# stardist/stardist

Hardware: AMD Instinct MI355X
Metric: predict_instances() Mpix/s (2D) + Mvox/s (3D) end-to-end at 1/2/4/8 GPU (higher is better)
Workload: dtype f32

## Files before the change

stardist_amd/csrc/clip_beam.h:

```cpp
#pragma once
#include "clip_sweep.h"
#include <limits.h>

#if defined(BEAM_COUNT) && !defined(__HIP_DEVICE_COMPILE__)
struct BeamCounters { long beams, topx, isect_pt, isect_edges, outpt, update, maxima, lm, horz, ael_sum, il_beams, es_loads; };
inline BeamCounters& beam_counters() { static BeamCounters c = {}; return c; }
#define BEAM_CNT(f, v) (beam_counters().f += (v))
#else
#define BEAM_CNT(f, v) ((void)0)
#endif
#ifndef BEAM_PH
#define BEAM_PH(i) ((void)0)
#endif
enum { BEAM_PH_PREP = 0, BEAM_PH_SETUP, BEAM_PH_LM, BEAM_PH_POP, BEAM_PH_HORZ, BEAM_PH_ILIST, BEAM_PH_ISECT, BEAM_PH_TOP_EDGES, BEAM_PH_TOP_HORZ,
       BEAM_PH_TOP_UPDATE, BEAM_PH_END, BEAM_PH_COUNT };

namespace sdclip {

typedef unsigned long long u64;

enum {
  ST_OVERFLOW_AEL = 32,
  ST_OVERFLOW_LM = 64,
  ST_OVERFLOW_GJ = 128
};
enum { BEAM_MAXLM = 8 };

struct PrepPt { int x, y; };
template <bool WIDE> struct PrepIdx { typedef unsigned char type; enum { NONE = 255 }; };
template <> struct PrepIdx<true> { typedef unsigned short type; enum { NONE = 65535 }; };
template <int MAXV>
struct PolyPrep {
  typedef typename PrepIdx<(MAXV > 128)>::type pidx;
  enum { NONE = PrepIdx<(MAXV > 128)>::NONE };
  int n;
  int n_lm;
  int status;
  int pad;
  PrepPt v[MAXV + 1];
  unsigned char ecode[MAXV];
  pidx mpair[MAXV];
  pidx hlast[MAXV];
  pidx lm_left[BEAM_MAXLM], lm_right[BEAM_MAXLM];
};

#ifndef BEAM_PREP_IDX
#define BEAM_PREP_IDX short
#endif
template <class P, int MAXV>
struct PrepWork {
  typedef BEAM_PREP_IDX ridx;
  static constexpr unsigned RI = P::template region<int, MAXV>(), RS = P::template region<ridx, MAXV>(),
                            RB = P::template region<unsigned char, MAXV>();
  static constexpr unsigned O_CX = 0, O_CY = O_CX + RI, O_NXT = O_CY + RI, O_PRV = O_NXT + RS, O_CODE = O_PRV + RS,
                            O_N = O_CODE + RB, O_LMY = O_N + P::template region<int, 1>(), O_LML = O_LMY + P::template region<int, BEAM_MAXLM>(),
                            O_LMR = O_LML + P::template region<short, BEAM_MAXLM>(), O_END = O_LMR + P::template region<short, BEAM_MAXLM>();
  static constexpr unsigned lds_bytes() { return O_END; }
  typename P::template Arr<int, MAXV, O_CX> cx; typename P::template Arr<int, MAXV, O_CY> cy;
  typename P::template Arr<ridx, MAXV, O_NXT> nxt; typename P::template Arr<ridx, MAXV, O_PRV> prv;
  typename P::template Arr<unsigned char, MAXV, O_CODE> code;
  typename P::template Scalar<int, O_N> n;
  typename P::template Arr<int, BEAM_MAXLM, O_LMY> lmy;
  typename P::template Arr<short, BEAM_MAXLM, O_LML> lml_; typename P::template Arr<short, BEAM_MAXLM, O_LMR> lmr_;

  SD_HD int nx(int e) const { return e + 1 == n ? 0 : e + 1; }
  SD_HD int pv(int e) const { return e == 0 ? n - 1 : e - 1; }
  SD_HD bool sw(int e) const { return (code[e] & 4) != 0; }
  SD_HD int botx(int e) const { return sw(e) ? cx[nx(e)] : cx[e]; }
  SD_HD int boty(int e) const { return sw(e) ? cy[nx(e)] : cy[e]; }
  SD_HD int topx(int e) const { return sw(e) ? cx[e] : cx[nx(e)]; }
  SD_HD int topy(int e) const { return sw(e) ? cy[e] : cy[nx(e)]; }
  SD_HD bool is_horz(int e) const { return cy[e] == cy[nx(e)]; }
  SD_HD double dx(int e) const {
    const i64 dy = (i64)topy(e) - boty(e);
    if (dy == 0) return SD_HORIZONTAL;
    return (double)((i64)topx(e) - botx(e)) / (double)dy;
// ... 136 lines not shown
      if (n_lm < BEAM_MAXLM) {
        int k = n_lm;
        while (k > 0 && lmy[k - 1] < y) { lmy[k] = lmy[k - 1]; lml_[k] = lml_[k - 1]; lmr_[k] = lmr_[k - 1]; --k; }
        lmy[k] = y; lml_[k] = (short)left; lmr_[k] = (short)right;
        ++n_lm;
      } else st |= ST_OVERFLOW_LM;
      if (!leftFwd) E = E2;
    }
    for (int i = 0; i < m; ++i) { out->v[i].x = cx[i]; out->v[i].y = cy[i]; }
    out->v[m].x = cx[0]; out->v[m].y = cy[0];
    for (int i = 0; i < m; ++i) {
      const int c = code[i] & 3;
      const int nl = (c == 1) ? nx(i) : (c == 2 ? pv(i) : -1);
      int cc = code[i] & 7;
      if (nl >= 0 && is_horz(nl)) cc |= 8;
      out->ecode[i] = (unsigned char)cc;
      const int a = nx(i), b = pv(i);
      int mp = PolyPrep<MAXV>::NONE;
      if (topx(a) == topx(i) && topy(a) == topy(i) && (code[a] & 3) == 0) mp = a;
      else if (topx(b) == topx(i) && topy(b) == topy(i) && (code[b] & 3) == 0) mp = b;
      out->mpair[i] = (typename PolyPrep<MAXV>::pidx)mp;
      int last = i, g2 = 0;
      if (is_horz(i)) {
        for (;;) {
          const int c2 = code[last] & 3;
          const int n2 = (c2 == 1) ? nx(last) : (c2 == 2 ? pv(last) : -1);
          if (n2 < 0 || !is_horz(n2)) break;
          last = n2;
          if (++g2 > MAXV) { st |= ST_ITER; break; }
        }
      }
      out->hlast[i] = (typename PolyPrep<MAXV>::pidx)last;
    }
    for (int i = 0; i < n_lm; ++i) { out->lm_left[i] = (typename PolyPrep<MAXV>::pidx)lml_[i]; out->lm_right[i] = (typename PolyPrep<MAXV>::pidx)lmr_[i]; }
    out->n = m; out->n_lm = n_lm; out->status = st;
  }
};

template <class D, class P, int MAXV, int K, int MAXIL, bool FULLGJ = false>
struct BeamCore {
  typedef PolyPrep<MAXV> Prep;
  template <bool W, int = 0> struct OrdT { typedef unsigned int type; };
  template <int D0> struct OrdT<true, D0> { typedef u64 type; };
  typedef typename OrdT<(K > 8)>::type ord_t;
  enum { ORD_BITS = (K > 8) ? 64 : 32 };
  enum { GJ = (K <= 8 ? 3 : 4), NX = (K <= 8 ? 2 : 4), EID_POLY = 4096 };
  SD_HD D& self() { return *static_cast<D*>(this); }
  static constexpr unsigned RI = P::template coord_region<K>(), RD = P::template slope_region<K>(),
                            RS = P::template region<short, K>(), RB = P::template region<signed char, K>(),
                            RIL = P::template coord_region<MAXIL>(), RILB = P::template region<signed char, MAXIL>(),
                            RG = P::template coord_region<GJ>(), RGF = P::template region<int, (FULLGJ ? GJ : 1)>(), R1 = P::template region<int, 1>(), R8 = P::template region<u64, 1>(), RO = P::template region<ord_t, 1>();
  static constexpr unsigned O_BOTX = 0, O_BOTY = O_BOTX + RI, O_TOPX = O_BOTY + RI, O_TOPY = O_TOPX + RI, O_CURX = O_TOPY + RI,
                            O_DX = O_CURX + RI, O_EID = O_DX + RD, O_WCNT = O_EID + RS, O_WCNT2 = O_WCNT + RB,
                            O_OUTIDX = O_WCNT2 + RB, O_LMLC = O_OUTIDX + RB, O_WDELTA = O_LMLC + RB, O_PTYP = O_WDELTA + RB,
                            O_SIDE = O_PTYP + RB, O_ILX = O_SIDE + RB, O_ILY = O_ILX + RIL, O_ILE1 = O_ILY + RIL, O_ILE2 = O_ILE1 + RILB,
                            O_GJOP = O_ILE2 + RILB, O_GJX1 = O_GJOP + RGF, O_GJX2 = O_GJX1 + RG, O_GJY2 = O_GJX2 + RG,
                            O_XTRA = O_GJY2 + RGF, O_MLM = O_XTRA + P::template region<int, NX>(),
                            O_PA = O_MLM + P::template region<unsigned char, 16>(),
                            O_ORD = O_PA + 2 * R8, O_HSEL = O_ORD + RO, O_AFTER_ORD = O_HSEL + RO, O_PB = O_PA + R8, O_NAEL = O_AFTER_ORD, O_FREE = O_NAEL + R1, O_NLM = O_FREE + R1,
                            O_CURLM = O_NLM + R1, O_NIL = O_CURLM + R1, O_STATUS = O_NIL + R1, O_NJOINS = O_STATUS + R1,
                            O_NGJ = O_NJOINS + R1, O_NXTRA = O_NGJ + R1, O_LMY = O_NXTRA + R1, O_ORGX = O_LMY + R1, O_ORGY = O_ORGX + R1, O_SCANY = O_ORGY + R1, O_RINGN = O_SCANY + R1,
                            O_CORE_END = O_RINGN + P::template region<int, 2>();
  typename P::template CoordArr<K, O_BOTX, O_ORGX, O_STATUS> botx; typename P::template CoordArr<K, O_BOTY, O_ORGY, O_STATUS> boty;
  typename P::template CoordArr<K, O_TOPX, O_ORGX, O_STATUS> topx; typename P::template CoordArr<K, O_TOPY, O_ORGY, O_STATUS> topy;
  typename P::template CoordArr<K, O_CURX, O_ORGX, O_STATUS> curx;
  typename P::template SlopeArr<K, O_DX, O_BOTX, O_BOTY, O_TOPX, O_TOPY> dx;
  typename P::template Arr<short, K, O_EID> eid;
  typename P::template Arr<signed char, K, O_WCNT> wcnt; typename P::template Arr<signed char, K, O_WCNT2> wcnt2;
  typename P::template Arr<signed char, K, O_OUTIDX> outidx;
  typename P::template Arr<signed char, K, O_LMLC> lmlc;
  typename P::template Arr<signed char, K, O_WDELTA> wdelta; typename P::template Arr<signed char, K, O_PTYP> ptyp;
  typename P::template Arr<signed char, K, O_SIDE> side;
  typename P::template CoordArr<MAXIL, O_ILX, O_ORGX, O_STATUS> ilx; typename P::template CoordArr<MAXIL, O_ILY, O_ORGY, O_STATUS> ily;
  typename P::template Arr<signed char, MAXIL, O_ILE1> ile1; typename P::template Arr<signed char, MAXIL, O_ILE2> ile2;
  typename P::template Arr<int, (FULLGJ ? GJ : 1), O_GJOP> gjop; typename P::template CoordArr<GJ, O_GJX1, O_ORGX, O_STATUS> gjx1;
  typename P::template CoordArr<GJ, O_GJX2, O_ORGX, O_STATUS> gjx2; typename P::template Arr<int, (FULLGJ ? GJ : 1), O_GJY2> gjy2;
  typename P::template Arr<int, NX, O_XTRA> xtra;
  typename P::template Arr<unsigned char, 16, O_MLM> mlm;
  typename P::template Scalar<ord_t, O_ORD> ord;
  typename P::template Scalar<ord_t, O_HSEL> hsel;
  typename P::template Scalar<const Prep*, O_PA> prepA; typename P::template Scalar<const Prep*, O_PB> prepB;
  typename P::template Scalar<int, O_NAEL> n_ael; typename P::template Scalar<int, O_FREE> freemask;
  typename P::template Scalar<int, O_NLM> n_lm; typename P::template Scalar<int, O_CURLM> cur_lm;
  typename P::template Scalar<int, O_NIL> n_il; typename P::template Scalar<int, O_STATUS> status;
  typename P::template Scalar<int, O_NJOINS> n_joins; typename P::template Scalar<int, O_NGJ> n_gj;
  typename P::template Scalar<int, O_NXTRA> n_xtra;
  typename P::template Scalar<int, O_LMY> next_lm_y;
  typename P::template Scalar<int, O_ORGX> orgx; typename P::template Scalar<int, O_ORGY> orgy;
  typename P::template Scalar<int, O_SCANY> scan_y;
  typename P::template Arr<int, 2, O_RINGN> ring_n;

  static constexpr ord_t ALLF = (ord_t)~(ord_t)0;
  static constexpr ord_t ONES = (ord_t)0x1111111111111111ull, HIGHS = (ord_t)0x8888888888888888ull;
  static SD_HD int nib(ord_t w, int p) { return (int)((w >> (4 * p)) & (ord_t)15); }
  static SD_HD int nib_find(ord_t w, int h) {
    const ord_t x = w ^ ((ord_t)h * ONES);
    const ord_t t = (ord_t)(x - ONES) & ~x & HIGHS;
    if (!t) return -1;
#if defined(__HIP_DEVICE_COMPILE__)
    return (ORD_BITS == 64) ? ((__ffsll((long long)t) - 1) >> 2) : ((__ffs((int)t) - 1) >> 2);
#else
    return (ORD_BITS == 64) ? (__builtin_ctzll((u64)t) >> 2) : (__builtin_ctz((unsigned)t) >> 2);
#endif
  }
  static SD_HD ord_t nib_insert(ord_t w, int p, int h) {
    const ord_t lowmask = (p == 0) ? (ord_t)0 : (ord_t)(ALLF >> (ORD_BITS - 4 * p));
    return (ord_t)((w & lowmask) | ((ord_t)h << (4 * p)) | ((ord_t)(w & ~lowmask) << 4));
  }
  static SD_HD ord_t nib_remove(ord_t w, int p) {
    const ord_t lowmask = (p == 0) ? (ord_t)0 : (ord_t)(ALLF >> (ORD_BITS - 4 * p));
    return (ord_t)((w & lowmask) | (((w >> 4) & ~lowmask)) | ((ord_t)0xF << (ORD_BITS - 4)));
  }
  static SD_HD ord_t nib_swap(ord_t w, int p, int q) {
// ... 17 lines not shown
  }

  SD_HD const Prep* prep_of(int id) const { return (id >= EID_POLY) ? (const Prep*)prepB : (const Prep*)prepA; }
  static SD_HD int ring_nx(int n, int i) { return i + 1 == n ? 0 : i + 1; }
  static SD_HD int ring_pv(int n, int i) { return i == 0 ? n - 1 : i - 1; }
  struct ES { int bx, by, tx, ty, code; };
  static SD_HD ES edge_static(const Prep* q, int i) {
    BEAM_CNT(es_loads, 1);
    ES s;
    s.code = q->ecode[i];
    const PrepPt p0 = q->v[i], p1 = q->v[i + 1];
    const int x0 = p0.x, y0 = p0.y, x1 = p1.x, y1 = p1.y;
    if (s.code & 4) { s.bx = x1; s.by = y1; s.tx = x0; s.ty = y0; }
    else { s.bx = x0; s.by = y0; s.tx = x1; s.ty = y1; }
    return s;
  }
  SD_HD int lml_id(int id, int code) const {
    const int c = code & 3;
    if (!c) return -1;
    const int n = ring_n[id >= EID_POLY ? 1 : 0];
    const int base = id & ~(EID_POLY - 1), i = id & (EID_POLY - 1);
    return base + (c == 1 ? ring_nx(n, i) : ring_pv(n, i));
  }
  SD_HD ES es_of(int id) const { return edge_static(prep_of(id), id & (EID_POLY - 1)); }
  static SD_HD double es_dx(const ES& s) {
    const i64 dy = (i64)s.ty - s.by;
    if (dy == 0) return SD_HORIZONTAL;
    return (double)((i64)s.tx - s.bx) / (double)dy;
  }
  SD_HD void load_slot(int h, int id) {
    const ES s = es_of(id);
    botx[h] = s.bx; boty[h] = s.by; topx[h] = s.tx; topy[h] = s.ty;
    dx[h] = es_dx(s);
    eid[h] = (short)id; lmlc[h] = (signed char)(s.code & 11);
  }

  SD_HD bool is_horz(int h) const { return topy[h] == boty[h]; }
  SD_HD i64 top_x(int h, i64 y) const {
    BEAM_CNT(topx, 1);
    return (y == topy[h]) ? (i64)topx[h] : (i64)botx[h] + sd_round(dx[h] * (double)(y - boty[h]));
  }
  static SD_HD bool slopes_equal4(i64 x1, i64 y1, i64 x2, i64 y2, i64 x3, i64 y3, i64 x4, i64 y4) {
    return (y1 - y2) * (x3 - x4) == (x1 - x2) * (y3 - y4);
  }
  SD_HD bool slopes_equal_e(int e1, int e2) const {
    return ((i64)topy[e1] - boty[e1]) * ((i64)topx[e2] - botx[e2]) ==
           ((i64)topx[e1] - botx[e1]) * ((i64)topy[e2] - boty[e2]);
  }
  static SD_HD bool horz_segments_overlap(i64 a1, i64 a2, i64 b1, i64 b2) {
    if (a1 > a2) { i64 t = a1; a1 = a2; a2 = t; }
    if (b1 > b2) { i64 t = b1; b1 = b2; b2 = t; }
    return (a1 < b2) && (b1 < a2);
  }
  SD_HD void add_join(int op1, int op2, int offx, int offy) { ++n_joins; self().out_add_join(op1, op2, offx, offy); }
  SD_HD void add_ghost_join(int op, int x1, int x2, int y2) {
    const int g = n_gj;
    if (g < GJ) { gjop[FULLGJ ? g : 0] = op; gjx1[g] = x1; gjx2[g] = x2; gjy2[FULLGJ ? g : 0] = y2; n_gj = g + 1; }
    else { ++n_joins; status |= ST_OVERFLOW_GJ; }
  }
  SD_HD void horz_joins(int horz, int op1) {
    ord_t w = hsel;
    for (int h = (int)(w & 15u); h != 15; w = (ord_t)((w >> 4) | ((ord_t)0xF << (ORD_BITS - 4))), h = (int)(w & 15u))
      if (outidx[h] >= 0 && horz_segments_overlap(botx[horz], topx[horz], botx[h], topx[h]))
        add_join(self().out_last_pt(h), op1, topx[h], topy[h]);
  }
  SD_HD void push_xtra(int y) {
    const int k = n_xtra;
    for (int i = 0; i < k; ++i) if (xtra[i] == y) return;
    if (k < NX) { xtra[k] = y; n_xtra = k + 1; } else status |= ST_OVERFLOW_GJ;
  }
  SD_HD int lm_y(int i) const {
    const int m = mlm[i];
    const Prep* q = (m & 128) ? (const Prep*)prepB : (const Prep*)prepA;
    const int l = q->lm_left[m & 127];
    const ES s = edge_static(q, l);
    return s.by;
  }
  SD_HD bool pop_scanbeam(int curY, int& y) {
    bool have = false; int best = 0;
    if (cur_lm < n_lm) { best = next_lm_y; have = true; }
    const int k = n_xtra;
    for (int i = 0; i < k; ++i) { const int v = xtra[i]; if (!have || v > best) { best = v; have = true; } }
    const ord_t w = ord; const int n = n_ael;
    for (int p = 0; p < n; ++p) {
      const int h = nib(w, p);
      const int t = topy[h];
      if (t != boty[h] && t < curY && (!have || t > best)) { best = t; have = true; }
    }
    if (!have) return false;
    int kk = 0;
    for (int i = 0; i < k; ++i) { const int v = xtra[i]; if (v != best) { xtra[kk] = v; ++kk; } }
    n_xtra = kk;
    y = best;
    return true;
  }

  template <bool IN> SD_HD int add_out_pt_t(int e, int px, int py) {
    BEAM_CNT(outpt, 1);
    if (IN) return self().out_add_pt_i(e, px, py);
    return self().out_add_pt(e, px, py);
  }
  SD_HD int add_out_pt(int e, int px, int py) { return add_out_pt_t<false>(e, px, py); }
  template <bool IN> SD_HD void add_local_max_poly_t(int e1, int e2, int px, int py) {
    add_out_pt_t<IN>(e1, px, py);
    if (outidx[e1] == outidx[e2]) {
      if (outidx[e1] >= 0) self().out_ring_closed(outidx[e1]);
      outidx[e1] = kUnassigned; outidx[e2] = kUnassigned;
    } else if (self().out_ring_before(outidx[e1], outidx[e2])) { if (IN) self().out_append_i(e1, e2); else self().out_append(e1, e2); }
    else { if (IN) self().out_append_i(e2, e1); else self().out_append(e2, e1); }
  }
  SD_HDN void add_local_max_poly(int e1, int e2, int px, int py) { add_local_max_poly_t<true>(e1, e2, px, py); }
  SD_HDN int add_local_min_poly(int e1, int e2, int px, int py) { return add_local_min_poly_t<true>(e1, e2, px, py); }
  template <bool IN> SD_HD int add_local_min_poly_t(int e1, int e2, int px, int py) {
    int e, prevE, result;
    if (is_horz(e2) || dx[e1] > dx[e2]) {
      result = add_out_pt_t<IN>(e1, px, py);
      outidx[e2] = outidx[e1];
      side[e1] = kLeft; side[e2] = kRight;
      e = e1;
      prevE = (aprev(e) == e2) ? aprev(e2) : aprev(e);
    } else {
// ... 23 lines not shown
  SD_HDN void insert_edge_into_ael(int edge, int startEdge) {
    const int n = n_ael;
    ord_t w = ord;
    int at;
    if (n == 0) at = 0;
    else if (startEdge < 0 && e2_inserts_before_e1(nib(w, 0), edge)) at = 0;
    else {
      int p = (startEdge < 0) ? 0 : nib_find(w, startEdge);
      if (p < 0) p = 0;
      while (p + 1 < n && !e2_inserts_before_e1(nib(w, p + 1), edge)) ++p;
      at = p + 1;
    }
    ord = nib_insert(w, at, edge);
    n_ael = n + 1;
  }
  SD_HD void delete_from_ael(int e) {
    const ord_t w = ord;
    const int p = nib_find(w, e);
    if (p < 0) return;
    ord = nib_remove(w, p);
    n_ael = n_ael - 1;
    freemask = freemask | (1 << e);
  }
  SD_HD void swap_positions_in_ael(int e1, int e2) {
    const ord_t w = ord;
    const int p = nib_find(w, e1), q = nib_find(w, e2);
    if (p < 0 || q < 0) return;
    ord = nib_swap(w, p, q);
  }
  SD_HD void add_edge_to_sel(int edge) { hsel = (ord_t)(((ord_t)hsel << 4) | (ord_t)edge); }
  SD_HDN int update_edge_into_ael(int e) {
    BEAM_CNT(update, 1);
    const int id = eid[e];
    const int n = lml_id(id, lmlc[e]);
    if (n < 0) { status |= ST_FAIL; return e; }
    load_slot(e, n);
    curx[e] = botx[e];
    return e;
  }

  SD_HDN void set_winding_count(int edge) {
    const ord_t w = ord;
    const int pe = nib_find(w, edge);
    int p = pe - 1;
    while (p >= 0 && (ptyp[nib(w, p)] != ptyp[edge] || wdelta[nib(w, p)] == 0)) --p;
    if (p < 0) {
      wcnt[edge] = wdelta[edge];
      wcnt2[edge] = 0;
      p = 0;
    } else {
      const int e = nib(w, p);
      if (wcnt[e] * wdelta[e] < 0) {
        int a = wcnt[e] < 0 ? -wcnt[e] : wcnt[e];
        if (a > 1) {
          if (wdelta[e] * wdelta[edge] < 0) wcnt[edge] = wcnt[e];
          else wcnt[edge] = (signed char)(wcnt[e] + wdelta[edge]);
        } else wcnt[edge] = (wdelta[edge] == 0 ? 1 : wdelta[edge]);
      } else {
        if (wdelta[edge] == 0) wcnt[edge] = (signed char)(wcnt[e] < 0 ? wcnt[e] - 1 : wcnt[e] + 1);
        else if (wdelta[e] * wdelta[edge] < 0) wcnt[edge] = wcnt[e];
        else wcnt[edge] = (signed char)(wcnt[e] + wdelta[edge]);
      }
      wcnt2[edge] = wcnt2[e];
      ++p;
    }
    for (; p < pe; ++p) wcnt2[edge] = (signed char)(wcnt2[edge] + wdelta[nib(w, p)]);
  }
// ... 20 lines not shown
        add_local_max_poly_t<true>(e1, e2, px, py);
      } else {
        add_out_pt_t<true>(e1, px, py);
        add_out_pt_t<true>(e2, px, py);
        signed char s = side[e1]; side[e1] = side[e2]; side[e2] = s;
        signed char o = outidx[e1]; outidx[e1] = outidx[e2]; outidx[e2] = o;
      }
    } else if (c1) {
      if (e2Wc == 0 || e2Wc == 1) {
        add_out_pt_t<true>(e1, px, py);
        signed char s = side[e1]; side[e1] = side[e2]; side[e2] = s;
        signed char o = outidx[e1]; outidx[e1] = outidx[e2]; outidx[e2] = o;
      }
    } else if (c2) {
      if (e1Wc == 0 || e1Wc == 1) {
        add_out_pt_t<true>(e2, px, py);
        signed char s = side[e1]; side[e1] = side[e2]; side[e2] = s;
        signed char o = outidx[e1]; outidx[e1] = outidx[e2]; outidx[e2] = o;
      }
    } else if ((e1Wc == 0 || e1Wc == 1) && (e2Wc == 0 || e2Wc == 1)) {
      int e1Wc2 = wcnt2[e1] < 0 ? -wcnt2[e1] : wcnt2[e1];
      int e2Wc2 = wcnt2[e2] < 0 ? -wcnt2[e2] : wcnt2[e2];
      if (ptyp[e1] != ptyp[e2]) add_local_min_poly_t<true>(e1, e2, px, py);
      else if (e1Wc == 1 && e2Wc == 1) {
        if (e1Wc2 > 0 && e2Wc2 > 0) add_local_min_poly_t<true>(e1, e2, px, py);
      } else { signed char s = side[e1]; side[e1] = side[e2]; side[e2] = s; }
    }
  }

  SD_BLK void insert_local_minima_into_ael(int botY) {
    while (cur_lm < n_lm && next_lm_y == botY) {
      const int m = mlm[cur_lm];
      ++cur_lm;
      if (cur_lm < n_lm) next_lm_y = lm_y(cur_lm);
      BEAM_CNT(lm, 1);
      const int poly = (m & 128) ? 1 : 0;
      const Prep* q = poly ? (const Prep*)prepB : (const Prep*)prepA;
      const int li = q->lm_left[m & 127], ri = q->lm_right[m & 127];
      const int lb = alloc_slot();
      const int rb = alloc_slot();
      if (status & ST_OVERFLOW_AEL) return;
      load_slot(lb, poly * EID_POLY + li);
      load_slot(rb, poly * EID_POLY + ri);
      const signed char wl = (ring_nx(ring_n[poly], li) == ri) ? -1 : 1;
      wdelta[lb] = wl; wdelta[rb] = (signed char)-wl;
      const signed char pt = poly ? (signed char)kSubject : (signed char)kClip;
      ptyp[lb] = pt; ptyp[rb] = pt;
      curx[lb] = botx[lb]; side[lb] = kLeft; outidx[lb] = kUnassigned; wcnt[lb] = 0; wcnt2[lb] = 0;
      curx[rb] = botx[rb]; side[rb] = kRight; outidx[rb] = kUnassigned; wcnt[rb] = 0; wcnt2[rb] = 0;

      int op1 = -1; bool have_op1 = false;
      insert_edge_into_ael(lb, -1);
      insert_edge_into_ael(rb, lb);
      set_winding_count(lb);
      wcnt[rb] = wcnt[lb]; wcnt2[rb] = wcnt2[lb];
      if (is_contributing(lb)) { op1 = add_local_min_poly(lb, rb, botx[lb], boty[lb]); have_op1 = true; }
      if (is_horz(rb)) {
        add_edge_to_sel(rb);
        const int nid = lml_id(eid[rb], lmlc[rb]);
        if (nid >= 0) push_xtra(es_of(nid).ty);
      }
      if (is_horz(lb)) status |= ST_ITER;

      if (have_op1 && is_horz(rb) && n_gj > 0 && wdelta[rb] != 0) {
        const int ng = n_gj;
        for (int g = 0; g < ng; ++g)
          if (horz_segments_overlap(gjx1[g], gjx2[g], botx[rb], topx[rb])) add_join(gjop[FULLGJ ? g : 0], op1, gjx2[g], gjy2[FULLGJ ? g : 0]);
      }
      const int lp = aprev(lb);
      if (outidx[lb] >= 0 && lp >= 0 && curx[lp] == botx[lb] && outidx[lp] >= 0 &&
          slopes_equal4(botx[lp], boty[lp], topx[lp], topy[lp], curx[lb], scan_y, topx[lb], topy[lb]) &&
          wdelta[lb] != 0 && wdelta[lp] != 0) {
        const int op2 = add_out_pt(lp, botx[lb], boty[lb]);
        add_join(op1, op2, topx[lb], topy[lb]);
      }
      if (anext(lb) != rb) {
        const int rp = aprev(rb);
        if (outidx[rb] >= 0 && rp >= 0 && outidx[rp] >= 0 &&
            slopes_equal4(curx[rp], scan_y, topx[rp], topy[rp], curx[rb], scan_y, topx[rb], topy[rb]) &&
            wdelta[rb] != 0 && wdelta[rp] != 0) {
          const int op2 = add_out_pt(rp, botx[rb], boty[rb]);
          add_join(op1, op2, topx[rb], topy[rb]);
        }
        int e = anext(lb);
        int guard = 0;
        while (e >= 0 && e != rb) {
          intersect_edges(rb, e, curx[lb], scan_y);
          e = anext(e);
          if (++guard > K) { status |= ST_ITER; break; }
        }
      }
    }
// ... 12 lines not shown
  SD_HD int get_maxima_pair_ex(int e, int& slot) const {
    slot = -1;
    const int r = get_maxima_pair_id(eid[e]);
    if (r < 0) return -1;
    slot = slot_of(r);
    if (slot < 0) {
      const ES s = es_of(r);
      if (s.ty != s.by) return -1;
    }
    return r;
  }
  SD_BLK void process_horizontal(int horz) {
    BEAM_CNT(horz, 1);
    bool l2r; i64 hl, hr;
    if (botx[horz] < topx[horz]) { hl = botx[horz]; hr = topx[horz]; l2r = true; }
    else { hl = topx[horz]; hr = botx[horz]; l2r = false; }
    int eLast, eMaxPair = -1;
    {
      const int id = eid[horz];
      const Prep* q = prep_of(id);
      const int base = id & ~(EID_POLY - 1);
      const int li = q->hlast[id & (EID_POLY - 1)];
      eLast = base + li;
      if ((q->ecode[li] & 3) == 0) { const int mp = q->mpair[li]; if (mp != Prep::NONE) eMaxPair = base + mp; }
    }
    int op1 = -1; bool have_op1 = false;
    int guard = 0;
    for (;;) {
      const bool isLast = (eid[horz] == eLast);
      int e = l2r ? anext(horz) : aprev(horz);
      while (e >= 0) {
        if (++guard > 4 * K * K + 4 * MAXV) { status |= ST_ITER; return; }
        if ((l2r && curx[e] > hr) || (!l2r && curx[e] < hl)) break;
        if (curx[e] == topx[horz] && (lmlc[horz] & 3) != 0) {
          const ES s = es_of(lml_id(eid[horz], lmlc[horz]));
          if (dx[e] < es_dx(s)) break;
        }
        if (outidx[horz] >= 0) {
          op1 = add_out_pt(horz, curx[e], scan_y);
          have_op1 = true;
          horz_joins(horz, op1);
          add_ghost_join(op1, curx[e], botx[horz], boty[horz]);
        }
        if (eid[e] == eMaxPair && isLast) {
          if (outidx[horz] >= 0) add_local_max_poly(horz, e, topx[horz], topy[horz]);
          delete_from_ael(horz);
          delete_from_ael(e);
          return;
        }
        if (l2r) intersect_edges(horz, e, curx[e], scan_y);
        else intersect_edges(e, horz, curx[e], scan_y);
        const int eNext = l2r ? anext(e) : aprev(e);
        swap_positions_in_ael(horz, e);
        e = eNext;
      }
      if ((lmlc[horz] & 8) == 0) break;
      horz = update_edge_into_ael(horz);
      if (outidx[horz] >= 0) add_out_pt(horz, botx[horz], boty[horz]);
      if (botx[horz] < topx[horz]) { hl = botx[horz]; hr = topx[horz]; l2r = true; }
      else { hl = topx[horz]; hr = botx[horz]; l2r = false; }
    }
    if (outidx[horz] >= 0 && !have_op1) {
      op1 = self().out_last_pt(horz);
      horz_joins(horz, op1);
      add_ghost_join(op1, self().out_last_pt_x(horz), topx[horz], topy[horz]);
    }
    if ((lmlc[horz] & 3) != 0) {
      if (outidx[horz] >= 0) {
        op1 = add_out_pt(horz, topx[horz], topy[horz]);
        horz = update_edge_into_ael(horz);
        if (wdelta[horz] == 0) return;
        const int ePrev = aprev(horz), eNext = anext(horz);
        if (ePrev >= 0 && curx[ePrev] == botx[horz] && scan_y == boty[horz] && wdelta[ePrev] != 0 &&
            (outidx[ePrev] >= 0 && scan_y > topy[ePrev] && slopes_equal_e(horz, ePrev))) {
          const int op2 = add_out_pt(ePrev, botx[horz], boty[horz]);
          add_join(op1, op2, topx[horz], topy[horz]);
        } else if (eNext >= 0 && curx[eNext] == botx[horz] && scan_y == boty[horz] && wdelta[eNext] != 0 &&
                   outidx[eNext] >= 0 && scan_y > topy[eNext] && slopes_equal_e(horz, eNext)) {
          const int op2 = add_out_pt(eNext, botx[horz], boty[horz]);
          add_join(op1, op2, topx[horz], topy[horz]);
        }
      } else update_edge_into_ael(horz);
    } else {
      if (outidx[horz] >= 0) add_out_pt(horz, topx[horz], topy[horz]);
      delete_from_ael(horz);
    }
  }
  SD_HD void process_horizontals() {
    int guard = 0;
    for (;;) {
      const ord_t w = hsel;
      const int h = (int)(w & 15u);
      if (h == 15) break;
      hsel = (ord_t)((w >> 4) | ((ord_t)0xF << (ORD_BITS - 4)));
      process_horizontal(h);
      if (++guard > 4 * MAXV) { status |= ST_ITER; break; }
    }
  }

  SD_HDN void intersect_point(int e1, int e2, i64& ipx, i64& ipy) const {
// ... 73 lines not shown
          const int pj = nib_find(w, ile1[j]), qj = nib_find(w, ile2[j]);
          if (pj - qj == 1 || qj - pj == 1) break;
          j++;
        }
        if (j == n) return false;
        const int y = ily[i], x = ilx[i]; const signed char a = ile1[i], b = ile2[i];
        ily[i] = ily[j]; ilx[i] = ilx[j]; ile1[i] = ile1[j]; ile2[i] = ile2[j];
        ily[j] = y; ilx[j] = x; ile1[j] = a; ile2[j] = b;
        p = nib_find(w, ile1[i]); q = nib_find(w, ile2[i]);
      }
      w = nib_swap(w, p, q);
    }
    return true;
  }
  SD_HD bool process_intersections(int topY) {
    if (n_ael == 0) return true;
    n_il = 0;
    build_intersect_list(topY);
    BEAM_PH(BEAM_PH_ILIST);
    const int n = n_il;
    if (n == 0) return true;
    BEAM_CNT(il_beams, 1); BEAM_CNT(isect_pt, n);
    if (n == 1 || fixup_intersection_order()) {
      for (int i = 0; i < n; ++i) {
        const int e1 = ile1[i], e2 = ile2[i];
        intersect_edges(e1, e2, ilx[i], ily[i]);
        swap_positions_in_ael(e1, e2);
      }
      n_il = 0;
    } else return false;
    return true;
  }

  SD_BLK void do_maxima(int e) {
    BEAM_CNT(maxima, 1);
    int mp;
    const int mpid = get_maxima_pair_ex(e, mp);
    if (mpid < 0) {
      if (outidx[e] >= 0) add_out_pt(e, topx[e], topy[e]);
      delete_from_ael(e);
      return;
    }
    if (mp < 0) { status |= ST_FAIL; return; }
    int eNext = anext(e);
    int guard = 0;
    while (eNext >= 0 && eNext != mp) {
      intersect_edges(e, eNext, topx[e], topy[e]);
      swap_positions_in_ael(e, eNext);
      eNext = anext(e);
      if (++guard > K) { status |= ST_ITER; break; }
    }
    if (outidx[e] == kUnassigned && outidx[mp] == kUnassigned) {
      delete_from_ael(e); delete_from_ael(mp);
    } else if (outidx[e] >= 0 && outidx[mp] >= 0) {
      add_local_max_poly(e, mp, topx[e], topy[e]);
      delete_from_ael(e); delete_from_ael(mp);
    } else status |= ST_FAIL;
  }
  SD_BLK void process_edges_at_top_of_scanbeam(int topY) {
    ord_t w = ord;
    int n = n_ael, p = 0;
    int guard = 0;
    while (p < n) {
      int e = nib(w, p);
      if (++guard > 4 * MAXV) { status |= ST_ITER; break; }
      bool isMax = (topy[e] == topY && (lmlc[e] & 3) == 0);
      if (isMax) {
        int mps;
        const int mp = get_maxima_pair_ex(e, mps);
        bool mpHorz = false;
        if (mp >= 0) { if (mps >= 0) mpHorz = is_horz(mps); else mpHorz = true; }
        isMax = (mp < 0 || !mpHorz);
      }
      if (isMax) {
        do_maxima(e);
        if (status & ST_FAIL) return;
        w = ord; n = n_ael;
      } else {
        if (topy[e] == topY && (lmlc[e] & 8) != 0) {
          e = update_edge_into_ael(e);
          if (outidx[e] >= 0) add_out_pt(e, botx[e], boty[e]);
          add_edge_to_sel(e);
        } else {
#if defined(BEAM_VERIFY_CURX) && !defined(__HIP_DEVICE_COMPILE__)
          { const int stored = curx[e]; curx[e] = (int)top_x(e, topY); sd_curx_checks()[0] += 1; sd_curx_checks()[1] += (stored != (int)curx[e]); }
#endif
        }
        ++p;
      }
    }
    scan_y = topY;
    BEAM_PH(BEAM_PH_TOP_EDGES);
    process_horizontals();
    BEAM_PH(BEAM_PH_TOP_HORZ);
    w = ord; n = n_ael;
    for (p = 0; p < n; ++p) {
      int e = nib(w, p);
      if (topy[e] == topY && (lmlc[e] & 3) != 0) {
        bool op = false; int oph = -1;
        if (outidx[e] >= 0) { oph = add_out_pt(e, topx[e], topy[e]); op = true; }
        e = update_edge_into_ael(e);
        const int ePrev = p > 0 ? nib(w, p - 1) : -1, eNext = p + 1 < n ? nib(w, p + 1) : -1;
        if (ePrev >= 0 && curx[ePrev] == botx[e] && scan_y == boty[e] && op &&
            outidx[ePrev] >= 0 && scan_y > topy[ePrev] &&
            slopes_equal4(curx[e], scan_y, topx[e], topy[e], curx[ePrev], scan_y, topx[ePrev], topy[ePrev]) &&
            wdelta[e] != 0 && wdelta[ePrev] != 0) {
          const int op2 = add_out_pt(ePrev, botx[e], boty[e]);
          add_join(oph, op2, topx[e], topy[e]);
        } else if (eNext >= 0 && curx[eNext] == botx[e] && scan_y == boty[e] && op &&
                   outidx[eNext] >= 0 && scan_y > topy[eNext] &&
                   slopes_equal4(curx[e], scan_y, topx[e], topy[e], curx[eNext], scan_y, topx[eNext], topy[eNext]) &&
                   wdelta[e] != 0 && wdelta[eNext] != 0) {
          const int op2 = add_out_pt(eNext, botx[e], boty[e]);
          add_join(oph, op2, topx[e], topy[e]);
        }
      }
    }
  }

  SD_HD void reset_core(const Prep* a, const Prep* b) {
    prepA = a; prepB = b; ring_n[0] = a->n; ring_n[1] = b->n;
    orgx = a->n ? a->v[0].x : (b->n ? b->v[0].x : 0); orgy = a->n ? a->v[0].y : (b->n ? b->v[0].y : 0);
    ord = ALLF; hsel = ALLF; n_ael = 0; freemask = (1 << K) - 1;
    n_lm = 0; cur_lm = 0; n_il = 0; status = ST_OK; n_joins = 0; n_gj = 0; n_xtra = 0;
  }
  SD_BLK bool run_sweep() {
    const Prep* a = prepA; const Prep* b = prepB;
    status |= (a->status | b->status);
    {
      const int na = a->n ? a->n_lm : 0, nb = b->n ? b->n_lm : 0;
      if (na + nb > 16) { status |= ST_OVERFLOW_LM; return false; }
      int ia = 0, ib = 0, k = 0;
      while (ia < na || ib < nb) {
        bool takeA;
        if (ia >= na) takeA = false;
        else if (ib >= nb) takeA = true;
        else takeA = edge_static(a, a->lm_left[ia]).by >= edge_static(b, b->lm_left[ib]).by;
        if (takeA) { mlm[k] = (unsigned char)ia; ++ia; } else { mlm[k] = (unsigned char)(128 + ib); ++ib; }
        ++k;
      }
      n_lm = k;
    }
    if (n_lm == 0) return true;
    cur_lm = 0;
    next_lm_y = lm_y(0);
    int botY = next_lm_y, topY = 0;
    scan_y = botY;
    BEAM_PH(BEAM_PH_SETUP);
    int guard = 0;
    bool ok = true;
    for (;;) {
      insert_local_minima_into_ael(botY);
      BEAM_PH(BEAM_PH_LM);
      if (status & (ST_OVERFLOW_AEL | ST_OVERFLOW_REC | ST_OVERFLOW_IL | ST_ITER)) { ok = false; break; }
      const bool popped = pop_scanbeam(botY, topY);
      BEAM_PH(BEAM_PH_POP);
      if (!popped) break;
      if (++guard > 4 * MAXV + 8) { status |= ST_ITER; break; }
      BEAM_CNT(beams, 1); BEAM_CNT(ael_sum, n_ael);
      process_horizontals();
      BEAM_PH(BEAM_PH_HORZ);
      n_gj = 0;
      const bool isect_ok = process_intersections(topY);
      BEAM_PH(BEAM_PH_ISECT);
      if (!isect_ok) { ok = false; break; }
      process_edges_at_top_of_scanbeam(topY);
      BEAM_PH(BEAM_PH_TOP_UPDATE);
      if (status & ST_FAIL) { ok = false; break; }
      botY = topY;
    }
// ... 108 lines not shown
```

stardist_amd/csrc/poly_pass.h:

```cpp
#pragma once
#include "clip_sweep.h"
#include "clip_beam.h"

namespace sdpass {

typedef long long i64;
constexpr int PASS_T = 64;
constexpr int PASS_V = 32;

SD_HD int px_(int p) { return (int)(short)(p & 0xffff); }
SD_HD int py_(int p) { return p >> 16; }
SD_HD int pack_(int x, int y) { return (int)(((unsigned)y << 16) | ((unsigned)x & 0xffffu)); }

struct FastPrep {
  const int* ring;
  int n;
  unsigned swm, l1m, l2m;

  SD_HD int P(int i) const { return ring[i * PASS_T]; }
  SD_HD int cx(int i) const { return px_(P(i)); }
  SD_HD int cy(int i) const { return py_(P(i)); }
  SD_HD int nx(int e) const { return e + 1 == n ? 0 : e + 1; }
  SD_HD int pv(int e) const { return e == 0 ? n - 1 : e - 1; }
  SD_HD bool sw(int e) const { return (swm >> e) & 1u; }
// ... 156 lines not shown
              for (int i = 0; i < sdclip::BEAM_MAXLM; ++i)
                if (i == k) { lmy[i] = y; lml[i] = left; lmr[i] = right; }
              ++n_lm;
            } else st |= sdclip::ST_OVERFLOW_LM;
            if (!leftFwd) E = E2;
          }
          for (int i = 0; i < m; ++i) { const int p = P(i); out->v[i].x = px_(p) + ox; out->v[i].y = py_(p) + oy; }
          out->v[m].x = cx(0) + ox; out->v[m].y = cy(0) + oy;
          for (int i = 0; i < m; ++i) {
            const int c = lmlc(i);
            const int nl = (c == 1) ? nx(i) : (c == 2 ? pv(i) : -1);
            int cc = c | (sw(i) ? 4 : 0);
            if (nl >= 0 && is_horz(nl)) cc |= 8;
            out->ecode[i] = (unsigned char)cc;
            const int a = nx(i), b = pv(i);
            int mp = Prep::NONE;
            if (topx(a) == topx(i) && topy(a) == topy(i) && lmlc(a) == 0) mp = a;
            else if (topx(b) == topx(i) && topy(b) == topy(i) && lmlc(b) == 0) mp = b;
            out->mpair[i] = (typename Prep::pidx)mp;
            int last = i, g2 = 0;
            if (is_horz(i)) {
              for (;;) {
                const int c2 = lmlc(last);
                const int n2 = (c2 == 1) ? nx(last) : (c2 == 2 ? pv(last) : -1);
                if (n2 < 0 || !is_horz(n2)) break;
                last = n2;
                if (++g2 > PASS_V) { st |= sdclip::ST_ITER; break; }
              }
            }
            out->hlast[i] = (typename Prep::pidx)last;
          }
#pragma unroll
          for (int i = 0; i < sdclip::BEAM_MAXLM; ++i)
            if (i < n_lm) { out->lm_left[i] = (typename Prep::pidx)lml[i]; out->lm_right[i] = (typename Prep::pidx)lmr[i]; }
        }
      } else m = 0;
    }
    if (m == 0) { n_lm = 0; st = 0; }
    out->n = m; out->n_lm = n_lm; out->status = st; out->pad = 0;
  }
};

}

#if defined(__HIPCC__)
#include <hip/hip_runtime.h>
#include "area_bounds.h"

namespace sdpass {

__device__ __forceinline__ sdarea::PolyProps props_pair(int X, int Y, bool cv, bool valid, int R, int l, int half, float2* sv) {
  using namespace sdarea;
  const int hb = half << 5;
  const int x0 = __shfl(X, hb), y0 = __shfl(Y, hb);
  const int xmin = half_min_i(valid ? X : 0x7fffffff), xmax = half_max_i(valid ? X : (int)0x80000000);
  const int ymin = half_min_i(valid ? Y : 0x7fffffff), ymax = half_max_i(valid ? Y : (int)0x80000000);
  const bool small = cv && (long long)xmax - xmin <= WINDOW && (long long)ymax - ymin <= WINDOW;
  const int ln = (l + 1 >= R) ? 0 : l + 1;
  const int rx = valid && small ? X - x0 : 0, ry = valid && small ? Y - y0 : 0;
  const int rbx = __shfl(rx, hb + ln), rby = __shfl(ry, hb + ln);
  const float ax = (float)rx, ay = (float)ry, bx = (float)rbx, by = (float)rby;
  const float ex = bx - ax, ey = by - ay;
  const bool deg = !valid || (ex == 0.f && ey == 0.f);
  const unsigned long long bal = __ballot(!deg);
  const unsigned int m32 = (unsigned int)(half ? (bal >> 32) : bal);
  const int count = __popc(m32);
  auto next_of = [&](int e) {
// ... 118 lines not shown
```

Before: 339.1.

## Pack per-edge codes into nibble word and iterate scanbeam tops via bitmasks

Replaces the per-slot lmlc byte array with a packed nibble word holding each active edge's local-min code plus a horizontal flag. Top-of-scanbeam processing now builds a bitmask of edges ending at topY and walks it with find-first-set, and pop_scanbeam scans all K slots in an unrolled loop. Local-minimum y values are precomputed into the prep struct so they no longer need an edge_static lookup. The aim is to cut scratch loads and branchy per-position checks in the beam sweep, at the cost of a larger prep struct and recomputing the position mask after each maxima deletion.

```diff
diff --git a/stardist_amd/csrc/clip_beam.h b/stardist_amd/csrc/clip_beam.h
--- a/stardist_amd/csrc/clip_beam.h
+++ b/stardist_amd/csrc/clip_beam.h
@@ -11,6 +11,11 @@
 #endif
 #ifndef BEAM_PH
 #define BEAM_PH(i) ((void)0)
+#endif
+enum { TOPS_POP = 0, TOPS_MASK, TOPS_WALK1, TOPS_WALK2, TOPS_LMY, TOPS_HORZ, TOPS_KINDS };
+#if defined(BEAM_VERIFY_TOPS) && !defined(__HIP_DEVICE_COMPILE__)
+inline long* sd_tops_checks() { static long c[2 * TOPS_KINDS] = {}; return c; }
+#define BEAM_TOPS_CHECK(kind, same) (sd_tops_checks()[2 * (kind)] += 1, sd_tops_checks()[2 * (kind) + 1] += ((same) ? 0 : 1))
 #endif
 enum { BEAM_PH_PREP = 0, BEAM_PH_SETUP, BEAM_PH_LM, BEAM_PH_POP, BEAM_PH_HORZ, BEAM_PH_ILIST, BEAM_PH_ISECT, BEAM_PH_TOP_EDGES, BEAM_PH_TOP_HORZ,
        BEAM_PH_TOP_UPDATE, BEAM_PH_END, BEAM_PH_COUNT };
@@ -42,6 +47,7 @@
   pidx mpair[MAXV];
   pidx hlast[MAXV];
   pidx lm_left[BEAM_MAXLM], lm_right[BEAM_MAXLM];
+  int lm_y[BEAM_MAXLM];
 };
 
 #ifndef BEAM_PREP_IDX
@@ -244,7 +250,7 @@
       }
       out->hlast[i] = (typename PolyPrep<MAXV>::pidx)last;
     }
-    for (int i = 0; i < n_lm; ++i) { out->lm_left[i] = (typename PolyPrep<MAXV>::pidx)lml_[i]; out->lm_right[i] = (typename PolyPrep<MAXV>::pidx)lmr_[i]; }
+    for (int i = 0; i < n_lm; ++i) { out->lm_left[i] = (typename PolyPrep<MAXV>::pidx)lml_[i]; out->lm_right[i] = (typename PolyPrep<MAXV>::pidx)lmr_[i]; out->lm_y[i] = lmy[i]; }
     out->n = m; out->n_lm = n_lm; out->status = st;
   }
 };
@@ -264,12 +270,12 @@
                             RG = P::template coord_region<GJ>(), RGF = P::template region<int, (FULLGJ ? GJ : 1)>(), R1 = P::template region<int, 1>(), R8 = P::template region<u64, 1>(), RO = P::template region<ord_t, 1>();
   static constexpr unsigned O_BOTX = 0, O_BOTY = O_BOTX + RI, O_TOPX = O_BOTY + RI, O_TOPY = O_TOPX + RI, O_CURX = O_TOPY + RI,
                             O_DX = O_CURX + RI, O_EID = O_DX + RD, O_WCNT = O_EID + RS, O_WCNT2 = O_WCNT + RB,
-                            O_OUTIDX = O_WCNT2 + RB, O_LMLC = O_OUTIDX + RB, O_WDELTA = O_LMLC + RB, O_PTYP = O_WDELTA + RB,
+                            O_OUTIDX = O_WCNT2 + RB, O_WDELTA = O_OUTIDX + RB, O_PTYP = O_WDELTA + RB,
                             O_SIDE = O_PTYP + RB, O_ILX = O_SIDE + RB, O_ILY = O_ILX + RIL, O_ILE1 = O_ILY + RIL, O_ILE2 = O_ILE1 + RILB,
                             O_GJOP = O_ILE2 + RILB, O_GJX1 = O_GJOP + RGF, O_GJX2 = O_GJX1 + RG, O_GJY2 = O_GJX2 + RG,
                             O_XTRA = O_GJY2 + RGF, O_MLM = O_XTRA + P::template region<int, NX>(),
                             O_PA = O_MLM + P::template region<unsigned char, 16>(),
-                            O_ORD = O_PA + 2 * R8, O_HSEL = O_ORD + RO, O_AFTER_ORD = O_HSEL + RO, O_PB = O_PA + R8, O_NAEL = O_AFTER_ORD, O_FREE = O_NAEL + R1, O_NLM = O_FREE + R1,
+                            O_ORD = O_PA + 2 * R8, O_HSEL = O_ORD + RO, O_CODES = O_HSEL + RO, O_AFTER_ORD = O_CODES + RO, O_PB = O_PA + R8, O_NAEL = O_AFTER_ORD, O_FREE = O_NAEL + R1, O_NLM = O_FREE + R1,
                             O_CURLM = O_NLM + R1, O_NIL = O_CURLM + R1, O_STATUS = O_NIL + R1, O_NJOINS = O_STATUS + R1,
                             O_NGJ = O_NJOINS + R1, O_NXTRA = O_NGJ + R1, O_LMY = O_NXTRA + R1, O_ORGX = O_LMY + R1, O_ORGY = O_ORGX + R1, O_SCANY = O_ORGY + R1, O_RINGN = O_SCANY + R1,
                             O_CORE_END = O_RINGN + P::template region<int, 2>();
@@ -280,7 +286,6 @@
   typename P::template Arr<short, K, O_EID> eid;
   typename P::template Arr<signed char, K, O_WCNT> wcnt; typename P::template Arr<signed char, K, O_WCNT2> wcnt2;
   typename P::template Arr<signed char, K, O_OUTIDX> outidx;
-  typename P::template Arr<signed char, K, O_LMLC> lmlc;
   typename P::template Arr<signed char, K, O_WDELTA> wdelta; typename P::template Arr<signed char, K, O_PTYP> ptyp;
   typename P::template Arr<signed char, K, O_SIDE> side;
   typename P::template CoordArr<MAXIL, O_ILX, O_ORGX, O_STATUS> ilx; typename P::template CoordArr<MAXIL, O_ILY, O_ORGY, O_STATUS> ily;
@@ -291,6 +296,7 @@
   typename P::template Arr<unsigned char, 16, O_MLM> mlm;
   typename P::template Scalar<ord_t, O_ORD> ord;
   typename P::template Scalar<ord_t, O_HSEL> hsel;
+  typename P::template Scalar<ord_t, O_CODES> codes;
   typename P::template Scalar<const Prep*, O_PA> prepA; typename P::template Scalar<const Prep*, O_PB> prepB;
   typename P::template Scalar<int, O_NAEL> n_ael; typename P::template Scalar<int, O_FREE> freemask;
   typename P::template Scalar<int, O_NLM> n_lm; typename P::template Scalar<int, O_CURLM> cur_lm;
@@ -374,10 +380,25 @@
     const ES s = es_of(id);
     botx[h] = s.bx; boty[h] = s.by; topx[h] = s.tx; topy[h] = s.ty;
     dx[h] = es_dx(s);
-    eid[h] = (short)id; lmlc[h] = (signed char)(s.code & 11);
-  }
-
-  SD_HD bool is_horz(int h) const { return topy[h] == boty[h]; }
+    eid[h] = (short)id;
+    const ord_t c = (ord_t)((s.code & 11) | (s.ty == s.by ? 4 : 0));
+    codes = (ord_t)(((ord_t)codes & ~((ord_t)15 << (4 * h))) | (c << (4 * h)));
+  }
+  SD_HD int code_of(int h) const { return nib(codes, h); }
+  SD_HD unsigned tops_at(int y) const {
+    unsigned m = 0;
+#pragma unroll
+    for (int h = 0; h < K; ++h) m |= (topy[h] == y ? 1u : 0u) << h;
+    return m;
+  }
+
+  SD_HD bool is_horz(int h) const {
+    const bool r = (code_of(h) & 4) != 0;
+#ifdef BEAM_TOPS_CHECK
+    BEAM_TOPS_CHECK(TOPS_HORZ, r == (topy[h] == boty[h]));
+#endif
+    return r;
+  }
   SD_HD i64 top_x(int h, i64 y) const {
     BEAM_CNT(topx, 1);
     return (y == topy[h]) ? (i64)topx[h] : (i64)botx[h] + sd_round(dx[h] * (double)(y - boty[h]));
@@ -414,21 +435,39 @@
   SD_HD int lm_y(int i) const {
     const int m = mlm[i];
     const Prep* q = (m & 128) ? (const Prep*)prepB : (const Prep*)prepA;
-    const int l = q->lm_left[m & 127];
-    const ES s = edge_static(q, l);
-    return s.by;
+    const int r = q->lm_y[m & 127];
+#ifdef BEAM_TOPS_CHECK
+    BEAM_TOPS_CHECK(TOPS_LMY, r == edge_static(q, q->lm_left[m & 127]).by);
+#endif
+    return r;
   }
   SD_HD bool pop_scanbeam(int curY, int& y) {
     bool have = false; int best = 0;
     if (cur_lm < n_lm) { best = next_lm_y; have = true; }
     const int k = n_xtra;
     for (int i = 0; i < k; ++i) { const int v = xtra[i]; if (!have || v > best) { best = v; have = true; } }
-    const ord_t w = ord; const int n = n_ael;
-    for (int p = 0; p < n; ++p) {
-      const int h = nib(w, p);
+    const ord_t cw = codes;
+    const unsigned taken = ~(unsigned)(int)freemask;
+#ifdef BEAM_TOPS_CHECK
+    bool have0 = have; int best0 = best;
+#endif
+#pragma unroll
+    for (int h = 0; h < K; ++h) {
       const int t = topy[h];
-      if (t != boty[h] && t < curY && (!have || t > best)) { best = t; have = true; }
-    }
+      const bool in = ((taken >> h) & 1u) != 0 && (nib(cw, h) & 4) == 0 && t < curY;
+      if (in && (!have || t > best)) { best = t; have = true; }
+    }
+#ifdef BEAM_TOPS_CHECK
+    {
+      const ord_t w = ord; const int n = n_ael;
+      for (int p = 0; p < n; ++p) {
+        const int h = nib(w, p);
+        const int t = topy[h];
+        if (t != boty[h] && t < curY && (!have0 || t > best0)) { best0 = t; have0 = true; }
+      }
+      BEAM_TOPS_CHECK(TOPS_POP, have == have0 && (!have || best == best0));
+    }
+#endif
     if (!have) return false;
     int kk = 0;
     for (int i = 0; i < k; ++i) { const int v = xtra[i]; if (v != best) { xtra[kk] = v; ++kk; } }
@@ -518,7 +557,7 @@
   SD_HDN int update_edge_into_ael(int e) {
     BEAM_CNT(update, 1);
     const int id = eid[e];
-    const int n = lml_id(id, lmlc[e]);
+    const int n = lml_id(id, code_of(e));
     if (n < 0) { status |= ST_FAIL; return e; }
     load_slot(e, n);
     curx[e] = botx[e];
@@ -605,7 +644,8 @@
     while (cur_lm < n_lm && next_lm_y == botY) {
       const int m = mlm[cur_lm];
       ++cur_lm;
-      if (cur_lm < n_lm) next_lm_y = lm_y(cur_lm);
+      const bool more = cur_lm < n_lm;
+      const int next_y = more ? lm_y(cur_lm) : 0;
       BEAM_CNT(lm, 1);
       const int poly = (m & 128) ? 1 : 0;
       const Prep* q = poly ? (const Prep*)prepB : (const Prep*)prepA;
@@ -615,6 +655,7 @@
       if (status & ST_OVERFLOW_AEL) return;
       load_slot(lb, poly * EID_POLY + li);
       load_slot(rb, poly * EID_POLY + ri);
+      if (more) next_lm_y = next_y;
       const signed char wl = (ring_nx(ring_n[poly], li) == ri) ? -1 : 1;
       wdelta[lb] = wl; wdelta[rb] = (signed char)-wl;
       const signed char pt = poly ? (signed char)kSubject : (signed char)kClip;
@@ -630,7 +671,7 @@
       if (is_contributing(lb)) { op1 = add_local_min_poly(lb, rb, botx[lb], boty[lb]); have_op1 = true; }
       if (is_horz(rb)) {
         add_edge_to_sel(rb);
-        const int nid = lml_id(eid[rb], lmlc[rb]);
+        const int nid = lml_id(eid[rb], code_of(rb));
         if (nid >= 0) push_xtra(es_of(nid).ty);
       }
       if (is_horz(lb)) status |= ST_ITER;
@@ -709,8 +750,8 @@
       while (e >= 0) {
         if (++guard > 4 * K * K + 4 * MAXV) { status |= ST_ITER; return; }
         if ((l2r && curx[e] > hr) || (!l2r && curx[e] < hl)) break;
-        if (curx[e] == topx[horz] && (lmlc[horz] & 3) != 0) {
-          const ES s = es_of(lml_id(eid[horz], lmlc[horz]));
+        if (curx[e] == topx[horz] && (code_of(horz) & 3) != 0) {
+          const ES s = es_of(lml_id(eid[horz], code_of(horz)));
           if (dx[e] < es_dx(s)) break;
         }
         if (outidx[horz] >= 0) {
@@ -731,7 +772,7 @@
         swap_positions_in_ael(horz, e);
         e = eNext;
       }
-      if ((lmlc[horz] & 8) == 0) break;
+      if ((code_of(horz) & 8) == 0) break;
       horz = update_edge_into_ael(horz);
       if (outidx[horz] >= 0) add_out_pt(horz, botx[horz], boty[horz]);
       if (botx[horz] < topx[horz]) { hl = botx[horz]; hr = topx[horz]; l2r = true; }
@@ -742,7 +783,7 @@
       horz_joins(horz, op1);
       add_ghost_join(op1, self().out_last_pt_x(horz), topx[horz], topy[horz]);
     }
-    if ((lmlc[horz] & 3) != 0) {
+    if ((code_of(horz) & 3) != 0) {
       if (outidx[horz] >= 0) {
         op1 = add_out_pt(horz, topx[horz], topy[horz]);
         horz = update_edge_into_ael(horz);
@@ -882,10 +923,8 @@
     return true;
   }
 
-  SD_BLK void do_maxima(int e) {
+  SD_BLK void do_maxima(int e, int mpid, int mp) {
     BEAM_CNT(maxima, 1);
-    int mp;
-    const int mpid = get_maxima_pair_ex(e, mp);
     if (mpid < 0) {
       if (outidx[e] >= 0) add_out_pt(e, topx[e], topy[e]);
       delete_from_ael(e);
@@ -907,36 +946,65 @@
       delete_from_ael(e); delete_from_ael(mp);
     } else status |= ST_FAIL;
   }
+  static SD_HD unsigned end_positions(ord_t w, int n, unsigned ends, ord_t cw, int from, bool second) {
+    unsigned pm = 0;
+    for (int p = from; p < n; ++p) {
+      const int e = nib(w, p), c = nib(cw, e);
+      const bool hit = ((ends >> e) & 1u) != 0 && (second ? (c & 3) != 0 : ((c & 3) == 0 || (c & 8) != 0));
+      pm |= (hit ? 1u : 0u) << p;
+    }
+    return pm;
+  }
   SD_BLK void process_edges_at_top_of_scanbeam(int topY) {
     ord_t w = ord;
     int n = n_ael, p = 0;
     int guard = 0;
-    while (p < n) {
+    unsigned ends = tops_at(topY);
+    ord_t cw = codes;
+#ifdef BEAM_TOPS_CHECK
+    { unsigned m0 = 0, in = 0; for (int q = 0; q < n; ++q) { const int h = nib(w, q); in |= 1u << h; if (topy[h] == topY) m0 |= 1u << h; } BEAM_TOPS_CHECK(TOPS_MASK, (ends & in) == m0); }
+    for (int q = 0; q < n; ++q) {
+      const int h = nib(w, q), c0 = es_of(eid[h]).code & 11, ch = nib(cw, h);
+      BEAM_TOPS_CHECK(TOPS_WALK1, (((ends >> h) & 1u) != 0) == (topy[h] == topY) && (ch & 11) == c0 && ((ch & 4) != 0) == (topy[h] == boty[h]));
+    }
+#endif
+#if defined(BEAM_VERIFY_CURX) && !defined(__HIP_DEVICE_COMPILE__)
+    for (int q = 0; q < n; ++q) {
+      const int h = nib(w, q), ch = nib(cw, h);
+      if (((ends >> h) & 1u) != 0 && ((ch & 3) == 0 || (ch & 8) != 0)) continue;
+      const int stored = curx[h]; curx[h] = (int)top_x(h, topY); sd_curx_checks()[0] += 1; sd_curx_checks()[1] += (stored != (int)curx[h]);
+    }
+#endif
+    unsigned pm = end_positions(w, n, ends, cw, 0, false);
+    while (pm) {
+#if defined(__HIP_DEVICE_COMPILE__)
+      p = __ffs((int)pm) - 1;
+#else
+      p = __builtin_ctz(pm);
+#endif
       int e = nib(w, p);
       if (++guard > 4 * MAXV) { status |= ST_ITER; break; }
-      bool isMax = (topy[e] == topY && (lmlc[e] & 3) == 0);
+      const int ce = nib(cw, e);
+      bool isMax = (ce & 3) == 0;
+      int mps = -1, mp = -1;
       if (isMax) {
-        int mps;
-        const int mp = get_maxima_pair_ex(e, mps);
+        mp = get_maxima_pair_ex(e, mps);
         bool mpHorz = false;
         if (mp >= 0) { if (mps >= 0) mpHorz = is_horz(mps); else mpHorz = true; }
         isMax = (mp < 0 || !mpHorz);
       }
       if (isMax) {
-        do_maxima(e);
+        do_maxima(e, mp, mps);
         if (status & ST_FAIL) return;
         w = ord; n = n_ael;
+        pm = end_positions(w, n, ends, cw, p, false);
       } else {
-        if (topy[e] == topY && (lmlc[e] & 8) != 0) {
+        if ((ce & 8) != 0) {
           e = update_edge_into_ael(e);
           if (outidx[e] >= 0) add_out_pt(e, botx[e], boty[e]);
           add_edge_to_sel(e);
-        } else {
-#if defined(BEAM_VERIFY_CURX) && !defined(__HIP_DEVICE_COMPILE__)
-          { const int stored = curx[e]; curx[e] = (int)top_x(e, topY); sd_curx_checks()[0] += 1; sd_curx_checks()[1] += (stored != (int)curx[e]); }
-#endif
         }
-        ++p;
+        pm &= pm - 1;
       }
     }
     scan_y = topY;
@@ -944,9 +1012,24 @@
     process_horizontals();
     BEAM_PH(BEAM_PH_TOP_HORZ);
     w = ord; n = n_ael;
-    for (p = 0; p < n; ++p) {
+    ends = tops_at(topY); cw = codes;
+#ifdef BEAM_TOPS_CHECK
+    { unsigned m0 = 0, in = 0; for (int q = 0; q < n; ++q) { const int h = nib(w, q); in |= 1u << h; if (topy[h] == topY) m0 |= 1u << h; } BEAM_TOPS_CHECK(TOPS_MASK, (ends & in) == m0); }
+#endif
+#ifdef BEAM_TOPS_CHECK
+    for (int q = 0; q < n; ++q) {
+      const int h = nib(w, q), c0 = es_of(eid[h]).code & 11;
+      BEAM_TOPS_CHECK(TOPS_WALK2, (((ends >> h) & 1u) != 0) == (topy[h] == topY) && (nib(cw, h) & 11) == c0);
+    }
+#endif
+    for (pm = end_positions(w, n, ends, cw, 0, true); pm; pm &= pm - 1) {
+#if defined(__HIP_DEVICE_COMPILE__)
+      p = __ffs((int)pm) - 1;
+#else
+      p = __builtin_ctz(pm);
+#endif
       int e = nib(w, p);
-      if (topy[e] == topY && (lmlc[e] & 3) != 0) {
+      {
         bool op = false; int oph = -1;
         if (outidx[e] >= 0) { oph = add_out_pt(e, topx[e], topy[e]); op = true; }
         e = update_edge_into_ael(e);
@@ -972,7 +1055,7 @@
     prepA = a; prepB = b; ring_n[0] = a->n; ring_n[1] = b->n;
     orgx = a->n ? a->v[0].x : (b->n ? b->v[0].x : 0); orgy = a->n ? a->v[0].y : (b->n ? b->v[0].y : 0);
     ord = ALLF; hsel = ALLF; n_ael = 0; freemask = (1 << K) - 1;
-    n_lm = 0; cur_lm = 0; n_il = 0; status = ST_OK; n_joins = 0; n_gj = 0; n_xtra = 0;
+    codes = 0; n_lm = 0; cur_lm = 0; n_il = 0; status = ST_OK; n_joins = 0; n_gj = 0; n_xtra = 0;
   }
   SD_BLK bool run_sweep() {
     const Prep* a = prepA; const Prep* b = prepB;
@@ -985,7 +1068,7 @@
         bool takeA;
         if (ia >= na) takeA = false;
         else if (ib >= nb) takeA = true;
-        else takeA = edge_static(a, a->lm_left[ia]).by >= edge_static(b, b->lm_left[ib]).by;
+        else takeA = a->lm_y[ia] >= b->lm_y[ib];
         if (takeA) { mlm[k] = (unsigned char)ia; ++ia; } else { mlm[k] = (unsigned char)(128 + ib); ++ib; }
         ++k;
       }
diff --git a/stardist_amd/csrc/poly_pass.h b/stardist_amd/csrc/poly_pass.h
--- a/stardist_amd/csrc/poly_pass.h
+++ b/stardist_amd/csrc/poly_pass.h
@@ -212,7 +212,7 @@
           }
 #pragma unroll
           for (int i = 0; i < sdclip::BEAM_MAXLM; ++i)
-            if (i < n_lm) { out->lm_left[i] = (typename Prep::pidx)lml[i]; out->lm_right[i] = (typename Prep::pidx)lmr[i]; }
+            if (i < n_lm) { out->lm_left[i] = (typename Prep::pidx)lml[i]; out->lm_right[i] = (typename Prep::pidx)lmr[i]; out->lm_y[i] = lmy[i] + oy; }
         }
       } else m = 0;
     }
```

Measured after the change: 342.9, median of 6. No clear change (+1.1%).
